# aspuru-guzik-group/waveflow

Hardware: AMD Instinct MI355X
Metric: flow log-prob evals/sec (higher is better)
Workload: dtype f32

## Files before the change

waveflow_amd/csrc/wf_kernels_scalar.hip:

```cpp
#include "wf_scalar_impl.h"

namespace wf {

namespace scalar {
WF_SCALAR_SHAPE(extern, 2, 32) WF_SCALAR_SHAPE(extern, 3, 32) WF_SCALAR_SHAPE(extern, 4, 32) WF_SCALAR_SHAPE(extern, 5, 32)
WF_SCALAR_SHAPE(extern, 6, 32) WF_SCALAR_SHAPE(extern, 7, 32) WF_SCALAR_SHAPE(extern, 8, 32)
WF_SCALAR_SHAPE(extern, 2, 64) WF_SCALAR_SHAPE(extern, 3, 64) WF_SCALAR_SHAPE(extern, 4, 64) WF_SCALAR_SHAPE(extern, 5, 64)
WF_SCALAR_SHAPE(extern, 6, 64) WF_SCALAR_SHAPE(extern, 7, 64) WF_SCALAR_SHAPE(extern, 8, 64)
}

namespace {
using namespace scalar;

constexpr int kSumBlock = 256;
constexpr int kSumMaxBlocks = 1024;

__device__ __forceinline__ void block_reduce2(double& a, double& b, double* sm) {
    sm[threadIdx.x] = a;
    sm[kSumBlock + threadIdx.x] = b;
    __syncthreads();
    for (int s = kSumBlock / 2; s > 0; s >>= 1) {
        if ((int)threadIdx.x < s) {
            sm[threadIdx.x] += sm[threadIdx.x + s];
            sm[kSumBlock + threadIdx.x] += sm[kSumBlock + threadIdx.x + s];
        }
        __syncthreads();
    }
    a = sm[0];
    b = sm[kSumBlock];
}

__device__ __forceinline__ void ring_push(double s, double q, double n, double* __restrict__ ring, int ring_len, unsigned long long* __restrict__ counter) {
    const unsigned long long c = *counter;
    double* slot = ring + (c % (unsigned long long)ring_len) * 3;
    slot[0] = s; slot[1] = q; slot[2] = n;
    *counter = c + 1;
}

__global__ __launch_bounds__(kSumBlock) void k_sums_stage1(const float* __restrict__ v, int64_t B, double* __restrict__ partial,
                                                           double* __restrict__ final, double* __restrict__ ring, int ring_len,
                                                           unsigned long long* __restrict__ counter) {
    __shared__ double sm[2 * kSumBlock];
    double s = 0.0, q = 0.0;
    for (int64_t i = (int64_t)blockIdx.x * kSumBlock + threadIdx.x; i < B; i += (int64_t)gridDim.x * kSumBlock) {
        const double x = (double)v[i];
        s += x;
        q += x * x;
    }
    block_reduce2(s, q, sm);
    if (threadIdx.x == 0) {
        if (final) {
            final[0] = s;
            final[1] = q;
            final[2] = (double)B;
            if (ring) ring_push(s, q, (double)B, ring, ring_len, counter);
        } else {
            partial[2 * blockIdx.x] = s;
            partial[2 * blockIdx.x + 1] = q;
        }
    }
}

__global__ __launch_bounds__(kSumBlock) void k_sums_stage2(const double* __restrict__ partial, int n_blocks, int64_t B, double* __restrict__ out,
                                                           double* __restrict__ ring, int ring_len, unsigned long long* __restrict__ counter) {
    __shared__ double sm[2 * kSumBlock];
    double s = 0.0, q = 0.0;
    for (int i = threadIdx.x; i < n_blocks; i += kSumBlock) {
        s += partial[2 * i];
        q += partial[2 * i + 1];
    }
    block_reduce2(s, q, sm);
    if (threadIdx.x == 0) {
        out[0] = s;
        out[1] = q;
        out[2] = (double)B;
        if (ring) ring_push(s, q, (double)B, ring, ring_len, counter);
    }
}

int sums_blocks(int64_t B) {
    int64_t n = (B + kSumBlock - 1) / kSumBlock;
    if (n < 1) n = 1;
    if (n > kSumMaxBlocks) n = kSumMaxBlocks;
    return (int)n;
}

int finish_launch() {
    hipError_t e = hipGetLastError();
    if (e != hipSuccess) {
        set_hip_error((int)e);
        return WF_ERR_HIP;
    }
    return WF_OK;
}

}

#define WF_DISPATCH_D(D_, NBP_, CALL)                                         \
    if ((NBP_) == 32) {                                                          \
        switch (D_) {                                                            \
            case 2: CALL(2, 32); break;                                          \
            case 3: CALL(3, 32); break;                                          \
            case 4: CALL(4, 32); break;                                          \
            case 5: CALL(5, 32); break;                                          \
            case 6: CALL(6, 32); break;                                          \
            case 7: CALL(7, 32); break;                                          \
            case 8: CALL(8, 32); break;                                          \
            default: return WF_ERR_UNSUPPORTED;                                  \
        }                                                                        \
    } else if ((NBP_) == 64) {                                                   \
        switch (D_) {                                                            \
            case 2: CALL(2, 64); break;                                          \
            case 3: CALL(3, 64); break;                                          \
            case 4: CALL(4, 64); break;                                          \
            case 5: CALL(5, 64); break;                                          \
            case 6: CALL(6, 64); break;                                          \
            case 7: CALL(7, 64); break;                                          \
            case 8: CALL(8, 64); break;                                          \
            default: return WF_ERR_UNSUPPORTED;                                  \
        }                                                                        \
    } else {                                                                     \
        return WF_ERR_UNSUPPORTED;                                               \
    }

int launch_scalar(const ModelDev& md, const ModelDev* md_dev, int mode, const float* x, int64_t B, float* out, float* u, int32_t* idx,
                  void* stream) {
    hipStream_t s = (hipStream_t)stream;
#define CALL(DD, NN) run_eval<DD, NN>(md_dev, mode, x, B, out, u, idx, s)
    WF_DISPATCH_D(md.D, md.nbp, CALL)
#undef CALL
    return finish_launch();
}

int launch_scalar_layer(const ModelDev& md, const ModelDev* md_dev, int layer, const float* u_in, int64_t B, float* y, float* logdet,
                        int32_t* idx, void* stream) {
    hipStream_t s = (hipStream_t)stream;
#define CALL(DD, NN) run_layer<DD, NN>(md_dev, layer, u_in, B, y, logdet, idx, s)
    WF_DISPATCH_D(md.D, md.nbp, CALL)
#undef CALL
    return finish_launch();
}

int launch_scalar_inverse(const ModelDev& md, const ModelDev* md_dev, const float* u, int64_t B, float* x, int exact, void* stream) {
    hipStream_t s = (hipStream_t)stream;
#define CALL(DD, NN) run_inverse<DD, NN>(md_dev, u, B, x, exact, s)
    WF_DISPATCH_D(md.D, md.nbp, CALL)
#undef CALL
    return finish_launch();
}

int launch_scalar_sample(const ModelDev& md, const ModelDev* md_dev, unsigned long long seed, int64_t B, float* x, float* latent, int exact,
                         void* stream) {
    hipStream_t s = (hipStream_t)stream;
#define CALL(DD, NN) run_sample<DD, NN>(md_dev, seed, B, x, latent, exact, s)
    WF_DISPATCH_D(md.D, md.nbp, CALL)
#undef CALL
    return finish_launch();
}

__global__ void k_sort_rows(const float* __restrict__ x, int64_t B, int D, float* __restrict__ xs, int32_t* __restrict__ inv) {
    const int64_t b = (int64_t)blockIdx.x * blockDim.x + threadIdx.x;
    if (b >= B) return;
    float r[WF_MAX_DIM];
    for (int d = 0; d < D; ++d) r[d] = x[b * D + d];
    int n = 0;
    for (int pass = 0; pass < D; ++pass)
        for (int i = pass & 1; i + 1 < D; i += 2)
            if (r[i] > r[i + 1]) {
                const float t = r[i]; r[i] = r[i + 1]; r[i + 1] = t;
                ++n;
            }
    if (xs)
        for (int d = 0; d < D; ++d) xs[b * D + d] = r[d];
    if (inv) inv[b] = n;
}
__global__ void k_apply_sign(float* __restrict__ v, const int32_t* __restrict__ inv, int64_t B) {
    const int64_t b = (int64_t)blockIdx.x * blockDim.x + threadIdx.x;
    if (b < B && (inv[b] & 1)) v[b] = -v[b];
}

int launch_sort_rows(const float* x, int64_t B, int D, float* xs, int32_t* inv, void* stream) {
    if (B <= 0) return WF_OK;
    hipLaunchKernelGGL(k_sort_rows, dim3((unsigned)((B + 255) / 256)), dim3(256), 0, (hipStream_t)stream, x, B, D, xs, inv);
    return finish_launch();
}
int launch_apply_sign(float* v, const int32_t* inv, int64_t B, void* stream) {
    if (B <= 0) return WF_OK;
    hipLaunchKernelGGL(k_apply_sign, dim3((unsigned)((B + 255) / 256)), dim3(256), 0, (hipStream_t)stream, v, inv, B);
    return finish_launch();
}

int64_t block_sums_ws_bytes(int64_t) { return (int64_t)kSumMaxBlocks * 2 * sizeof(double); }

int launch_block_sums(const float* v, int64_t B, double* out, void* ws, int64_t, void* stream, double* ring, int ring_len,
                      unsigned long long* counter) {
    hipStream_t s = (hipStream_t)stream;
    const int nb = sums_blocks(B);
    double* partial = (double*)ws;
    if (nb == 1) {
        hipLaunchKernelGGL(k_sums_stage1, dim3(1), dim3(kSumBlock), 0, s, v, B, partial, out, ring, ring_len, counter);
        return finish_launch();
    }
    hipLaunchKernelGGL(k_sums_stage1, dim3(nb), dim3(kSumBlock), 0, s, v, B, partial, (double*)nullptr, (double*)nullptr, 0,
                       (unsigned long long*)nullptr);
    hipLaunchKernelGGL(k_sums_stage2, dim3(1), dim3(kSumBlock), 0, s, (const double*)partial, nb, B, out, ring, ring_len, counter);
    return finish_launch();
}

}
```

Before: 4.271 billion.

## Fuse two-stage block sum reduction into single kernel with last-block ticket

Replaces the two-launch block-sum reduction with a single launch where each block writes its partial sums, takes an atomic ticket, and the last block to finish performs the final reduction and resets the ticket. A per-device, per-stream ticket table is allocated lazily on the host, with a fallback to the old two-kernel path during stream capture or on per-thread streams. This removes one kernel launch and the gap between the two launches, at the cost of an atomic plus fences per block and host-side map lookups under a mutex on every call.

```diff
diff --git a/waveflow_amd/csrc/wf_kernels_scalar.hip b/waveflow_amd/csrc/wf_kernels_scalar.hip
--- a/waveflow_amd/csrc/wf_kernels_scalar.hip
+++ b/waveflow_amd/csrc/wf_kernels_scalar.hip
@@ -1,3 +1,7 @@
+#include <map>
+#include <mutex>
+#include <unordered_map>
+
 #include "wf_scalar_impl.h"
 
 namespace wf {
@@ -37,37 +41,12 @@
     *counter = c + 1;
 }
 
-__global__ __launch_bounds__(kSumBlock) void k_sums_stage1(const float* __restrict__ v, int64_t B, double* __restrict__ partial,
-                                                           double* __restrict__ final, double* __restrict__ ring, int ring_len,
-                                                           unsigned long long* __restrict__ counter) {
-    __shared__ double sm[2 * kSumBlock];
-    double s = 0.0, q = 0.0;
-    for (int64_t i = (int64_t)blockIdx.x * kSumBlock + threadIdx.x; i < B; i += (int64_t)gridDim.x * kSumBlock) {
-        const double x = (double)v[i];
-        s += x;
-        q += x * x;
-    }
-    block_reduce2(s, q, sm);
-    if (threadIdx.x == 0) {
-        if (final) {
-            final[0] = s;
-            final[1] = q;
-            final[2] = (double)B;
-            if (ring) ring_push(s, q, (double)B, ring, ring_len, counter);
-        } else {
-            partial[2 * blockIdx.x] = s;
-            partial[2 * blockIdx.x + 1] = q;
-        }
-    }
-}
-
-__global__ __launch_bounds__(kSumBlock) void k_sums_stage2(const double* __restrict__ partial, int n_blocks, int64_t B, double* __restrict__ out,
-                                                           double* __restrict__ ring, int ring_len, unsigned long long* __restrict__ counter) {
-    __shared__ double sm[2 * kSumBlock];
+__device__ __forceinline__ void sums_finish(const double* partial, int n_blocks, int64_t B, double* __restrict__ out, double* __restrict__ ring,
+                                            int ring_len, unsigned long long* __restrict__ counter, double* sm) {
     double s = 0.0, q = 0.0;
     for (int i = threadIdx.x; i < n_blocks; i += kSumBlock) {
-        s += partial[2 * i];
-        q += partial[2 * i + 1];
+        s += __hip_atomic_load(partial + 2 * i, __ATOMIC_RELAXED, __HIP_MEMORY_SCOPE_AGENT);
+        q += __hip_atomic_load(partial + 2 * i + 1, __ATOMIC_RELAXED, __HIP_MEMORY_SCOPE_AGENT);
     }
     block_reduce2(s, q, sm);
     if (threadIdx.x == 0) {
@@ -76,6 +55,51 @@
         out[2] = (double)B;
         if (ring) ring_push(s, q, (double)B, ring, ring_len, counter);
     }
+}
+
+__global__ __launch_bounds__(kSumBlock) void k_sums_stage1(const float* __restrict__ v, int64_t B, double* partial, double* __restrict__ out,
+                                                           unsigned int* ticket, double* __restrict__ ring, int ring_len,
+                                                           unsigned long long* __restrict__ counter) {
+    __shared__ double sm[2 * kSumBlock];
+    __shared__ int is_last;
+    double s = 0.0, q = 0.0;
+    for (int64_t i = (int64_t)blockIdx.x * kSumBlock + threadIdx.x; i < B; i += (int64_t)gridDim.x * kSumBlock) {
+        const double x = (double)v[i];
+        s += x;
+        q += x * x;
+    }
+    block_reduce2(s, q, sm);
+    if (!ticket) {
+        if (threadIdx.x == 0) {
+            if (out) {
+                out[0] = s;
+                out[1] = q;
+                out[2] = (double)B;
+                if (ring) ring_push(s, q, (double)B, ring, ring_len, counter);
+            } else {
+                partial[2 * blockIdx.x] = s;
+                partial[2 * blockIdx.x + 1] = q;
+            }
+        }
+        return;
+    }
+    if (threadIdx.x == 0) {
+        partial[2 * blockIdx.x] = s;
+        partial[2 * blockIdx.x + 1] = q;
+        __threadfence();
+        is_last = atomicAdd(ticket, 1u) == gridDim.x - 1;
+    }
+    __syncthreads();
+    if (!is_last) return;
+    __threadfence();
+    sums_finish(partial, (int)gridDim.x, B, out, ring, ring_len, counter, sm);
+    if (threadIdx.x == 0) __hip_atomic_store(ticket, 0u, __ATOMIC_RELAXED, __HIP_MEMORY_SCOPE_AGENT);
+}
+
+__global__ __launch_bounds__(kSumBlock) void k_sums_stage2(const double* partial, int n_blocks, int64_t B, double* __restrict__ out,
+                                                           double* __restrict__ ring, int ring_len, unsigned long long* __restrict__ counter) {
+    __shared__ double sm[2 * kSumBlock];
+    sums_finish(partial, n_blocks, B, out, ring, ring_len, counter, sm);
 }
 
 int sums_blocks(int64_t B) {
@@ -192,17 +216,75 @@
 
 int64_t block_sums_ws_bytes(int64_t) { return (int64_t)kSumMaxBlocks * 2 * sizeof(double); }
 
+namespace {
+constexpr int kTicketSlots = 256;
+constexpr int kTicketStride = 16;
+
+struct TicketTable {
+    unsigned int* dev = nullptr;
+    std::unordered_map<hipStream_t, int> slot;
+};
+std::mutex g_ticket_mutex;
+std::map<int, TicketTable> g_ticket_tables;
+
+unsigned int* sums_ticket(hipStream_t s) {
+    if (s == hipStreamPerThread) return nullptr;
+    if (s != nullptr) {
+        hipStreamCaptureStatus cs = hipStreamCaptureStatusNone;
+        if (hipStreamIsCapturing(s, &cs) != hipSuccess) {
+            (void)hipGetLastError();
+            return nullptr;
+        }
+        if (cs != hipStreamCaptureStatusNone) return nullptr;
+    }
+    int dev = 0;
+    if (hipGetDevice(&dev) != hipSuccess) {
+        (void)hipGetLastError();
+        return nullptr;
+    }
+    std::lock_guard<std::mutex> lock(g_ticket_mutex);
+    TicketTable& t = g_ticket_tables[dev];
+    if (!t.dev) {
+        unsigned int* p = nullptr;
+        const size_t bytes = (size_t)kTicketSlots * kTicketStride * sizeof(unsigned int);
+        hipStreamCaptureMode mode = hipStreamCaptureModeRelaxed;
+        const bool exchanged = hipThreadExchangeStreamCaptureMode(&mode) == hipSuccess;
+        bool ok = hipMalloc((void**)&p, bytes) == hipSuccess;
+        if (ok && !(hipMemset(p, 0, bytes) == hipSuccess && hipDeviceSynchronize() == hipSuccess)) {
+            ok = false;
+            (void)hipFree(p);
+        }
+        if (exchanged) (void)hipThreadExchangeStreamCaptureMode(&mode);
+        if (!ok) {
+            (void)hipGetLastError();
+            return nullptr;
+        }
+        t.dev = p;
+    }
+    auto it = t.slot.find(s);
+    if (it == t.slot.end()) {
+        if ((int)t.slot.size() >= kTicketSlots) return nullptr;
+        it = t.slot.emplace(s, (int)t.slot.size()).first;
+    }
+    return t.dev + (size_t)it->second * kTicketStride;
+}
+}
+
 int launch_block_sums(const float* v, int64_t B, double* out, void* ws, int64_t, void* stream, double* ring, int ring_len,
                       unsigned long long* counter) {
     hipStream_t s = (hipStream_t)stream;
     const int nb = sums_blocks(B);
     double* partial = (double*)ws;
     if (nb == 1) {
-        hipLaunchKernelGGL(k_sums_stage1, dim3(1), dim3(kSumBlock), 0, s, v, B, partial, out, ring, ring_len, counter);
+        hipLaunchKernelGGL(k_sums_stage1, dim3(1), dim3(kSumBlock), 0, s, v, B, partial, out, (unsigned int*)nullptr, ring, ring_len, counter);
         return finish_launch();
     }
-    hipLaunchKernelGGL(k_sums_stage1, dim3(nb), dim3(kSumBlock), 0, s, v, B, partial, (double*)nullptr, (double*)nullptr, 0,
-                       (unsigned long long*)nullptr);
+    if (unsigned int* ticket = sums_ticket(s)) {
+        hipLaunchKernelGGL(k_sums_stage1, dim3(nb), dim3(kSumBlock), 0, s, v, B, partial, out, ticket, ring, ring_len, counter);
+        return finish_launch();
+    }
+    hipLaunchKernelGGL(k_sums_stage1, dim3(nb), dim3(kSumBlock), 0, s, v, B, partial, (double*)nullptr, (unsigned int*)nullptr,
+                       (double*)nullptr, 0, (unsigned long long*)nullptr);
     hipLaunchKernelGGL(k_sums_stage2, dim3(1), dim3(kSumBlock), 0, s, (const double*)partial, nb, B, out, ring, ring_len, counter);
     return finish_launch();
 }
```

New measurement: 3.967 billion. -7.1%, worse.
